# yardenas/ethz-safe-learning

Measured on NVIDIA B200. Metric: CEM-MPC plans/sec (PointGoal1 shape; ensemble transitions/sec alongside), higher is better.
Workload: dtype bf16

## Files before the change

ethz-safe-learning_b200/csrc/rollout_tc.cu:

```cuda
#include <cuda_bf16.h>

#include <cstdlib>
#include <type_traits>

#include "common.cuh"
#include "internal.h"
#include "rollout_params.cuh"
#include "tc_head.cuh"
#include "tc_ptx.cuh"

namespace simba {

#ifdef SIMBA_TC_TIMELINE
#define TL(ev)                                                                                   \
  do {                                                                                           \
    if (tl_who >= 0 && blockIdx.x == 0)                                                          \
      prm.timeline[(tl_who * 64 + tl_t) * 64 + (ev)] = clock64();  \
  } while (0)
#else
#define TL(ev) do { } while (0)
#endif

namespace {

constexpr int kU = 128;
constexpr int kMaxO = 60;
constexpr int kAtomBytes = 128 * 128;
constexpr int kBoundThreads = 640;

struct TileInfo {
  int32_t member, k0, count, valid;
};

template <int NB, int kThreads>
struct NoiseSmem {
  uint4* base;
  __device__ __forceinline__ uint4 get4(int b) const { return base[b * kThreads]; }
  __device__ __forceinline__ void put4(int b, uint4 v) { base[b * kThreads] = v; }
  __device__ __forceinline__ void put4_dyn(int b, uint4 v) { base[b * kThreads] = v; }
};
template <int NB>
struct NoiseRegs {
  uint4 v[NB];
  __device__ __forceinline__ uint4 get4(int b) const { return v[b]; }
  __device__ __forceinline__ void put4(int b, uint4 x) { v[b] = x; }
  __device__ __forceinline__ void put4_dyn(int b, uint4 x) {
#pragma unroll
    for (int i = 0; i < NB; ++i)
      if (i == b) v[i] = x;
  }
};

struct AStoreTmem {
  uint32_t t_a;
  __device__ __forceinline__ void store8(int k0, uint32_t p0, uint32_t p1, uint32_t p2, uint32_t p3) const {
    const uint32_t pk[4] = {p0, p1, p2, p3};
    tmem_st<4>(t_a + (uint32_t)(k0 >> 1), pk);
  }
};

struct AStorePair {
  uint32_t t_a;
  uint32_t peer_slot;
  uint32_t buf_off;
  uint32_t peer_bar;
  __device__ __forceinline__ void store8(int k0, uint32_t p0, uint32_t p1, uint32_t p2, uint32_t p3) const {
    const uint32_t pk[4] = {p0, p1, p2, p3};
    tmem_st<4>(t_a + (uint32_t)(k0 >> 1), pk);
    st_async_v4(peer_slot + buf_off, p0, p1, p2, p3, peer_bar);
  }
};

}

template <int NTILES, int Q, bool PAIR, bool TRAJ>
__device__ __forceinline__ void rollout_tc_body(const RolloutParams& prm) {
  static_assert(!PAIR || (NTILES == 1 && Q == 4), "the pair variant is the one-tile latency configuration");
  static_assert(!(PAIR && TRAJ), "the trajectory form has no pair variant");
  constexpr int kTileThreads = Q * 128;
  constexpr int kTileWarps = Q * 4;
  constexpr int kEpiThreads = NTILES * kTileThreads;
  constexpr int kEpiWarps = kEpiThreads / 32;
  constexpr int OW = (PAIR ? 32 : 64) / Q;
  constexpr int NSL = PAIR ? 2 * Q : Q;
  constexpr int NB = OW / 8;
  constexpr int HCOLS = 128 / Q;
  constexpr int kTmemCols = NTILES * 256;
  constexpr bool kPark = NTILES > 1;
  constexpr int kBarAcc = 2, kBarA = 2 + NTILES, kBarPart = 2 + 2 * NTILES, kBarFree = 2 + 3 * NTILES;
  extern __shared__ __align__(1024) uint8_t smem_raw[];
  const RowGeom& g = prm.g;
  const int L = prm.L;
  const int H = g.H;
  const int O = g.O, A = g.A;
  const int warp = threadIdx.x >> 5, lane = threadIdx.x & 31;
  const uint32_t crank = PAIR ? cluster_ctarank() : 0u;
  const int n_items = (prm.n_tiles + NTILES - 1) / NTILES;
  const int cta_item0 = PAIR ? (int)(blockIdx.x >> 1) : (int)blockIdx.x;
  const int n_ctas = PAIR ? (int)(gridDim.x >> 1) : (int)gridDim.x;
  const bool l0_pad_bias = (O + A + 2 <= 64);
  constexpr int n_quarters = 4;
  constexpr int tile_bar_threads = Q * 128 + 32;

  const uint32_t w_bytes = kAtomBytes + (uint32_t)L * 2 * kAtomBytes;
  uint8_t* w_smem = smem_raw;
  uint8_t* biask_smem = w_smem + w_bytes;
  uint8_t* ones_smem = biask_smem + (L + 1) * 4096;
  float* scale_smem = reinterpret_cast<float*>(ones_smem + 4096);
  float* pen_smem = scale_smem + 128;
  const int nparts = TRAJ ? 1 : 1 + prm.scorer.n_constraints;
  float* part_smem = pen_smem + kHeadParts * 64;
  const int part_buf_floats = NTILES * NSL * nparts * 128;
  uint4* xch_smem = reinterpret_cast<uint4*>(part_smem + (PAIR ? 2 : 1) * part_buf_floats);
  uint4* noise_smem = xch_smem + (PAIR ? 2 * Q * 128 : 0);
  uint32_t* rs_smem = reinterpret_cast<uint32_t*>(noise_smem + (kPark ? NB * kEpiThreads : 0));
  uint64_t* bars = reinterpret_cast<uint64_t*>(rs_smem + NTILES * 8 * 128);
  uint32_t* tmem_slot = reinterpret_cast<uint32_t*>(bars + 1 + NTILES + 2);
  TileInfo* tinfo = reinterpret_cast<TileInfo*>(tmem_slot + 2);
  uint64_t* seed_sh = reinterpret_cast<uint64_t*>(tinfo + NTILES);
  int32_t* w_state_sh = reinterpret_cast<int32_t*>(seed_sh + 1);

  const uint32_t bar_w = smem_u32(&bars[0]);

#ifdef SIMBA_TC_TIMELINE
#define TLK(k) do { if (blockIdx.x == 0 && threadIdx.x == 0) { prm.timeline[(3 * 64) * 64 + (k)] = clock64(); \
    unsigned long long gt_; asm volatile("mov.u64 %0, %%globaltimer;" : "=l"(gt_)); \
    prm.timeline[(3 * 64 + 10 + prm.iteration) * 64 + (k)] = (long long)gt_; } } while (0)
#else
#define TLK(k) do { } while (0)
#endif
  TLK(0);
  pdl_launch_dependents();
  auto item_member = [&](int item) {
    int wm = -1;
    for (int q = 0; q < NTILES; ++q)
      if (item * NTILES + q < prm.n_tiles && prm.tiles[item * NTILES + q].count > 0) wm = prm.tiles[item * NTILES + q].member;
    return wm;
  };
  auto stage_weights = [&](int wm) {
    const uint8_t* wsrc = reinterpret_cast<const uint8_t*>(prm.w_bf16) + (size_t)wm * prm.w_bf16_member_bytes;
    const uint32_t bk_bytes = (uint32_t)(L + 1) * 4096u;
    mbar_expect_tx(bar_w, w_bytes + bk_bytes);
    uint32_t off = 0;
    for (int l = 0; l <= L; ++l) {
      const uint32_t nb = (l == 0) ? kAtomBytes : 2 * kAtomBytes;
      bulk_g2s(smem_u32(w_smem + off), wsrc + off, nb, bar_w);
      off += nb;
    }
    bulk_g2s(smem_u32(biask_smem), reinterpret_cast<const uint8_t*>(prm.bias_k16) + (size_t)wm * bk_bytes,
             bk_bytes, bar_w);
    w_state_sh[0] = wm;
    w_state_sh[1] += 1;
  };
  if (threadIdx.x == 0) {
    mbar_init(bar_w, 1);
#pragma unroll
    for (int j = 0; j < NTILES; ++j) {
      mbar_init(smem_u32(&bars[1 + j]), 1);
    }
    if (PAIR) {
      mbar_init(smem_u32(&bars[1 + NTILES]), 1);
      mbar_init(smem_u32(&bars[2 + NTILES]), 1);
    }
    fence_barrier_init();
    w_state_sh[0] = -1;
    w_state_sh[1] = 0;
    const int wm = cta_item0 < n_items ? item_member(cta_item0) : -1;
    if (wm >= 0) stage_weights(wm);
  }
  auto load_tile = [&](int ti) {
    TileInfo info{0, 0, 0, 0};
    if (ti < prm.n_tiles) {
      const Tile t = prm.tiles[ti];
      info.member = t.member; info.k0 = t.k0; info.count = t.count;
      info.valid = t.count > 0 ? 1 : 0;
    }
    return info;
  };
  if (threadIdx.x < NTILES) tinfo[threadIdx.x] = load_tile(cta_item0 * NTILES + threadIdx.x);
  if (warp == 0) tmem_alloc(smem_u32(tmem_slot), kTmemCols);
  if (warp < kEpiWarps) {
    for (int i = threadIdx.x; i < 1024; i += kEpiThreads) {
      const int byte = i * 4;
      const bool first = ((byte & 255) < 128) && ((byte & 15) == 0);
      reinterpret_cast<uint32_t*>(ones_smem)[i] = first ? 0x3F803F80u : 0u;
    }
    fence_proxy_async();
    if constexpr (TRAJ) {
      head_tables_init(scale_smem, pen_smem, prm.tc_scale_a, prm.tc_scale_b, simba_scorer_t{},
                       l0_pad_bias ? O + A : -1, threadIdx.x, kEpiThreads);
    } else {
      head_tables_init(scale_smem, pen_smem, prm.tc_scale_a, prm.tc_scale_b, prm.scorer,
                       l0_pad_bias ? O + A : -1, threadIdx.x, kEpiThreads);
    }
  }
  if (PAIR && threadIdx.x == 0) {
    const uint32_t per_step = crank == 0 ? (uint32_t)(kEpiThreads * 4 * nparts) : 0u;
    mbar_expect_tx(smem_u32(&bars[2 + NTILES]), per_step + (uint32_t)(kEpiThreads * 16));
    const uint32_t b0 = per_step + (1 < H ? (uint32_t)(kEpiThreads * 16) : 0u);
    if (b0 != 0u) mbar_expect_tx(smem_u32(&bars[1 + NTILES]), b0);
  }
  tc_fence_before();
  __syncthreads();
  if (PAIR) cluster_sync_all();
  tc_fence_after();
  const uint32_t tmem_base = *tmem_slot;
  TLK(1);
  constexpr bool kLateWait = PAIR;
  if (!kLateWait) pdl_wait_prior_grid();
  TLK(2);
  if (threadIdx.x == 0) *seed_sh = prm.seed_ptr ? *prm.seed_ptr : prm.seed;
  auto tile_active = [&](const TileInfo& t) {
    if (prm.active == nullptr) return true;
    const int m = g.rows_per_state[t.member];
    bool any = false;
    for (int s = t.k0 / m; s <= (t.k0 + t.count - 1) / m; ++s) any = any || prm.active[s] != 0;
    return any;
  };
  auto late_gate = [&](const TileInfo& t) {
    if (!kLateWait) return true;
    pdl_wait_prior_grid();
    return tile_active(t);
  };
  uint32_t ph = 0;

#pragma unroll 1
  for (int item = cta_item0; item < n_items; item += n_ctas) {
  if (threadIdx.x < NTILES) {
    TileInfo info = tinfo[threadIdx.x];
    if (item != cta_item0) info = load_tile(item * NTILES + threadIdx.x);
    if (!kLateWait && info.valid) info.valid = tile_active(info) ? 1 : 0;
    tinfo[threadIdx.x] = info;
  }
  __syncthreads();
  bool any_valid = false;
  int member = -1;
#pragma unroll
  for (int j = 0; j < NTILES; ++j)
    if (tinfo[j].valid) { any_valid = true; member = tinfo[j].member; }
  if (threadIdx.x == 0 && any_valid && member != w_state_sh[0]) {
    if (w_state_sh[1] > 0) mbar_wait(bar_w, (uint32_t)(w_state_sh[1] - 1) & 1u);
    stage_weights(member);
  }
  __syncthreads();

  if (any_valid) {
    if (warp >= kEpiWarps + NTILES) {
      const int j = warp - kEpiWarps - NTILES;
      const TileInfo tis = tinfo[j];
      auto xbytes = [&](int t) -> uint32_t {
        return (crank == 0 ? (uint32_t)(kEpiThreads * 4 * nparts) : 0u) + (t + 1 < H ? (uint32_t)(kEpiThreads * 16) : 0u);
      };
      const uint32_t xbar = smem_u32(&bars[1 + NTILES]);
      if (PAIR && tis.valid && crank != 0 && late_gate(tis)) {
        for (int ts = -1; ts + 1 < H; ++ts) {
          mbar_wait(xbar + 8u * ((uint32_t)ts & 1u), (uint32_t)((ts + 1) >> 1) & 1u);
          if (lane == 0 && xbytes(ts + 2) != 0u) mbar_expect_tx(xbar + 8u * ((uint32_t)ts & 1u), xbytes(ts + 2));
        }
      }
      if (!TRAJ && tis.valid && crank == 0) {
        const simba_scorer_t& sc = prm.scorer;
        const bool done_first = objective_done_first(prm.objective);
        uint32_t* my_rs = rs_smem + j * 8 * 128 + lane;
        const float* part_tile0 = part_smem + (j * NSL * nparts) * 128;
#pragma unroll 1
        for (int i = 0; i < n_quarters; ++i) {
          const int row = lane + 32 * i;
#pragma unroll
          for (int f = 0; f < 7; ++f) my_rs[f * 128 + 32 * i] = 0u;
          my_rs[7 * 128 + 32 * i] = row < tis.count ? (uint32_t)decode_row(g, tis.member, tis.k0 + row).out : 0xffffffffu;
        }
        const bool live = late_gate(tis);
        for (int ts = -1; live && ts < H; ++ts) {
          named_bar_sync_n(kBarPart + j, tile_bar_threads);
          const float* part_tile = part_tile0;
          if (PAIR) {
            mbar_wait(xbar + 8u * ((uint32_t)ts & 1u), (uint32_t)((ts + 1) >> 1) & 1u);
            if (lane == 0 && ts + 2 < H) mbar_expect_tx(xbar + 8u * ((uint32_t)ts & 1u), xbytes(ts + 2));
            part_tile += (ts & 1) * part_buf_floats;
          }
#pragma unroll 1
          for (int i = 0; i < n_quarters; ++i) {
            uint32_t* q = my_rs + 32 * i;
            float nd, nc;
            head_combine<NSL>(sc, part_tile + lane + 32 * i, nparts, nd, nc);
            if (ts < 0) {
              q[4 * 128] = __float_as_uint(nd);
              q[5 * 128] = __float_as_uint(nc);
            } else {
              RowScore rs;
              rs.cum = __uint_as_float(q[0]);
              rs.costsum = __uint_as_float(q[128]);
              rs.cmask = (uint64_t)q[2 * 128] | ((uint64_t)q[3 * 128] << 32);
              rs.dist = __uint_as_float(q[4 * 128]);
              rs.cost = __uint_as_float(q[5 * 128]);
              rs.done = q[6 * 128] != 0u;
              head_score_step(rs, sc, done_first, ts, nd, nc);
              q[0] = __float_as_uint(rs.cum);
              q[128] = __float_as_uint(rs.costsum);
              q[2 * 128] = (uint32_t)rs.cmask;
              q[3 * 128] = (uint32_t)(rs.cmask >> 32);
              q[4 * 128] = __float_as_uint(rs.dist);
              q[5 * 128] = __float_as_uint(rs.cost);
              q[6 * 128] = rs.done ? 1u : 0u;
            }
          }
          if (ts + 1 < H) named_bar_arrive_n(kBarFree + j, tile_bar_threads);
        }
        if (live && prm.row_return != nullptr) {
#pragma unroll 1
          for (int i = 0; i < n_quarters; ++i) {
            const uint32_t* q = my_rs + 32 * i;
            const uint32_t slot = q[7 * 128];
            if (slot != 0xffffffffu) {
              prm.row_return[slot] = __uint_as_float(q[0]);
              prm.row_costmask[slot] = (uint64_t)q[2 * 128] | ((uint64_t)q[3 * 128] << 32);
              prm.row_costsum[slot] = __uint_as_float(q[128]);
            }
          }
        }
      }
    } else if (warp >= kEpiWarps) {
      const int j = warp - kEpiWarps;
      if (tinfo[j].valid) {
        const uint32_t bar_acc = smem_u32(&bars[1 + j]);
        const uint32_t d_tmem = tmem_base + (uint32_t)j * 128;
        const uint32_t a_tmem = tmem_base + (uint32_t)(NTILES * 192 + j * 64);
        const uint64_t ones_desc = umma_desc_k16_noswizzle(smem_u32(ones_smem));
        mbar_wait(bar_w, (uint32_t)(w_state_sh[1] - 1) & 1u);
#ifdef SIMBA_TC_TIMELINE
        const int tl_who = (j == 0 && lane == 0) ? 2 : -1;
#endif
        const bool live = late_gate(tinfo[j]);
        for (int t = 0; live && t < H; ++t) {
#ifdef SIMBA_TC_TIMELINE
          const int tl_t = t;
#endif
          for (int layer = 0; layer <= L; ++layer) {
            named_bar_sync_n(kBarA + j, tile_bar_threads);
            tc_fence_after();
            TL(2 * layer);
            if (elect_one()) {
              const uint32_t woff = (layer == 0) ? 0u : (uint32_t)(kAtomBytes + (layer - 1) * 2 * kAtomBytes);
              const uint64_t b0 = umma_desc_sw128(smem_u32(w_smem + woff));
#pragma unroll
              for (int k = 0; k < 4; ++k)
                umma_bf16_ts(d_tmem, a_tmem + (uint32_t)k * 8, b0 + (uint64_t)((k * 32) >> 4), kIdesc, k > 0 ? 1u : 0u);
              if (layer > 0) {
#pragma unroll
                for (int k = 4; k < 8; ++k)
                  umma_bf16_ts(d_tmem, a_tmem + (uint32_t)k * 8, b0 + (uint64_t)((kAtomBytes + (k - 4) * 32) >> 4),
                               kIdesc, 1u);
              }
              if (layer > 0 || !l0_pad_bias)
                umma_bf16(d_tmem, ones_desc, umma_desc_k16_noswizzle(smem_u32(biask_smem + layer * 4096)), kIdesc, 1u);
              umma_commit(bar_acc);
            }
            TL(2 * layer + 1);
            __syncwarp();
            mbar_wait(bar_acc, ph);
            ph ^= 1;
            tc_fence_before();
            named_bar_arrive_n(kBarAcc + j, tile_bar_threads);
          }
        }
      }
    } else {
      const int j = warp / kTileWarps;
      const int wl = warp - j * kTileWarps;
      const int cgp = wl >> 2;
      const int r = (wl & 3) * 32 + lane;
      const TileInfo ti = tinfo[j];
      if (ti.valid) {
        const bool row_ok = r < ti.count;
        const RowId id = decode_row(g, ti.member, ti.k0 + (row_ok ? r : 0));
        const uint32_t lane_base = tmem_base + ((uint32_t)((wl & 3) * 32) << 16);
        const uint32_t t_acc = lane_base + (uint32_t)j * 128;
        const uint32_t t_a = lane_base + (uint32_t)(NTILES * 192 + j * 64);
        const float* act_ptr = prm.actions + ((int64_t)id.s * g.N + id.i_global) * prm.action_stride;
        const simba_scorer_t& sc = prm.scorer;

        HeadCtx hc;
        hc.t_acc = t_acc;
        hc.t_state = lane_base + (uint32_t)(NTILES * 128 + j * 64);
        hc.o_base = (PAIR ? (int)crank * 32 : 0) + cgp * OW;
        hc.O = O; hc.A = A;
        hc.slice_bits = TRAJ ? 0u : head_slice_bits<OW>(sc, hc.o_base);
        hc.n_constraints = TRAJ ? 0 : sc.n_constraints;
        hc.scale_smem = scale_smem;
        hc.pen_smem = pen_smem;
        float* part_slot0 = part_smem + ((j * NSL + (int)crank * Q + cgp) * nparts) * 128 + r;
        hc.part = part_slot0 + (PAIR ? part_buf_floats : 0);
        typename std::conditional<PAIR, AStorePair, AStoreTmem>::type astore;
        astore.t_a = t_a;
        const uint32_t my_xbar = smem_u32(&bars[1 + NTILES]);
        const uint32_t peer_xbar = PAIR ? cluster_map_u32(my_xbar, crank ^ 1u) : 0u;
        const bool keeps_score = !TRAJ && (!PAIR || crank == 0);
        const uint32_t part_remote0 = (PAIR && crank != 0) ? cluster_map_u32(smem_u32(part_slot0), 0u) : 0u;
        if constexpr (PAIR) {
          astore.peer_slot = cluster_map_u32(smem_u32(xch_smem + cgp * 128 + r), crank ^ 1u);
          astore.buf_off = (uint32_t)(Q * 128 * sizeof(uint4));
          astore.peer_bar = peer_xbar + 8u;
          if (crank != 0) {
            hc.part_remote = part_remote0 + (uint32_t)(part_buf_floats * sizeof(float));
            hc.part_mbar = peer_xbar + 8u;
          }
        }
        auto exchange = [&](int t, bool next_step) {
          if constexpr (PAIR) {
            const uint32_t b = (uint32_t)t & 1u;
            if (next_step) {
              mbar_wait(my_xbar + 8u * b, (uint32_t)((t + 1) >> 1) & 1u);
              const uint4 v = xch_smem[(b * Q + cgp) * 128 + r];
              const uint32_t pk[4] = {v.x, v.y, v.z, v.w};
              tmem_st<4>(t_a + (uint32_t)((((int)crank ^ 1) * 32 + cgp * 8) >> 1), pk);
            }
          }
        };
        const float* s0_ptr = prm.states + (prm.state_per_row ? id.r_global : (int64_t)id.s) * prm.state_stride;
        typename std::conditional<TRAJ, TrajSink, NoTraj>::type sink{};
        if constexpr (TRAJ) {
          sink.row = row_ok ? prm.traj_out + id.out * (int64_t)(H + 1) * O : nullptr;
          sink.O = O;
        }

#ifdef SIMBA_TC_TIMELINE
        const int tl_who = (j == 0 && lane == 0) ? (wl == 0 ? 0 : (wl == kTileWarps - 1 ? 1 : -1)) : -1;
        int tl_t = 0;
#endif
        auto publish_a = [&]() {
          tmem_st_wait();
          tc_fence_before();
          named_bar_arrive_n(kBarA + j, tile_bar_threads);
        };
        auto wait_accumulator = [&]() {
          named_bar_sync_n(kBarAcc + j, tile_bar_threads);
          tc_fence_after();
        };

        const bool owns_actions = TRAJ ? (O < hc.o_base + OW) && (O + A > hc.o_base)
                                       : (O >= hc.o_base) && (O < hc.o_base + OW);
        float act_pf[4] = {0.f, 0.f, 0.f, 0.f};
        auto prefetch_actions = [&](int tn) {
          if (owns_actions && row_ok && tn < H) {
#pragma unroll
            for (int a = 0; a < 4; ++a)
              if (a < A) act_pf[a] = act_ptr[tn * A + a];
          }
        };

        typename std::conditional<kPark, NoiseSmem<NB, kEpiThreads>, NoiseRegs<NB>>::type noise;
        if constexpr (kPark) noise.base = noise_smem + threadIdx.x;
#pragma unroll
        for (int b = 0; b < NB; ++b) noise.put4(b, make_uint4(0u, 0u, 0u, 0u));
        const uint32_t c3_noise = (uint32_t)id.s | (kStreamNoise << 28);
        const uint32_t row32 = (uint32_t)id.r_global;
        const float* eps_row = prm.eps == nullptr ? nullptr
            : prm.eps + ((int64_t)id.s * H * ((int64_t)g.P * g.N) + id.r_global) * O;
        const int64_t eps_step = (int64_t)g.P * g.N * O;
        const uint64_t seed64 = *seed_sh;
        const uint2 key = make_uint2((uint32_t)seed64, (uint32_t)(seed64 >> 32));
        const uint32_t c2_base = (uint32_t)prm.iteration << 16;
        auto make_noise = [&](int b, int t) {
          const int o0 = hc.o_base + b * 8;
          if (o0 >= O) return;
          uint4 z;
          if (eps_row != nullptr) {
            z = external_noise8_bf16(eps_row + t * eps_step, o0, O);
          } else {
#ifdef SIMBA_TC_TIMELINE
            {
              PhiloxState p{(uint32_t)(o0 >> 3), row32, (uint32_t)t | c2_base, c3_noise, key.x, key.y};
              TL(50);
              philox_rounds<10>(p);
              if (p.c0 == 0x12345u) TL(53);
              TL(51);
              z = philox_finish_noise8_bf16(p);
              if (z.x == 0x12345u) TL(53);
              TL(52);
            }
#else
            z = philox_noise8_bf16(key, (uint32_t)(o0 >> 3), row32, (uint32_t)t | c2_base, c3_noise);
#endif
            if (o0 + 8 > O) z = mask_noise8(z, o0, O);
          }
          noise.put4_dyn(b, z);
        };
        float s0v[8];
        if constexpr (PAIR) {
#pragma unroll
          for (int i = 0; i < 8; ++i) s0v[i] = (row_ok && hc.o_base + i < O) ? s0_ptr[hc.o_base + i] : 0.0f;
        }
        const bool live = late_gate(ti);
        if (live) {
        prefetch_actions(0);
        if constexpr (PAIR) head_first_pass_vals(hc, astore, s0v, act_pf);
        else head_first_pass<OW>(hc, astore, s0_ptr, row_ok, act_pf, sink);
        prefetch_actions(1);
        exchange(-1, true);
        publish_a();
        TLK(3);
        if (keeps_score) named_bar_arrive_n(kBarPart + j, tile_bar_threads);

        PhiloxState ps{0u, 0u, 0u, 0u, 0u, 0u};
        for (int t = 0; t < H; ++t) {
#ifdef SIMBA_TC_TIMELINE
          tl_t = t;
#endif
          TL(0);
          if (owns_actions) {
            if constexpr (TRAJ) head_store_own_actions<OW>(hc, act_pf);
            else head_store_actions(hc, act_pf);
          }
          prefetch_actions(t + 2);
          for (int l = 0; l < L; ++l) {
            wait_accumulator();
            TL(1 + l * 4);
            {
              constexpr int NLD = HCOLS / 32;
              uint32_t v[NLD][32];
#pragma unroll
              for (int i = 0; i < NLD; ++i) tmem_ld<32>(t_acc + (uint32_t)(cgp * HCOLS + i * 32), v[i]);
              tmem_ld_wait();
#pragma unroll
              for (int i = 0; i < NLD; ++i) {
                uint32_t pk[16];
#pragma unroll
                for (int q = 0; q < 16; ++q)
                  pk[q] = pack_relu_bf16(__uint_as_float(v[i][2 * q]), __uint_as_float(v[i][2 * q + 1]));
                tmem_st<16>(t_a + (uint32_t)((cgp * HCOLS + i * 32) / 2), pk);
              }
            }
            TL(2 + l * 4);
            publish_a();
            TL(3 + l * 4);
            if (prm.sampling_propagation) {
              if (NTILES == 1 && L >= 2 * NB && eps_row == nullptr) {
                const int b = l >> 1, o0 = hc.o_base + b * 8;
                if (b < NB && o0 < O) {
                  if ((l & 1) == 0) {
                    ps = PhiloxState{(uint32_t)(o0 >> 3), row32, (uint32_t)t | c2_base, c3_noise, key.x, key.y};
                    philox_rounds<10>(ps);
                  } else {
                    uint4 z = philox_finish_noise8_bf16(ps);
                    if (o0 + 8 > O) z = mask_noise8(z, o0, O);
                    noise.put4_dyn(b, z);
                  }
                }
              } else {
                if (l < NB) make_noise(l, t);
                if (l == L - 1)
                  for (int b = L; b < NB; ++b) make_noise(b, t);
              }
            }
            TL(4 + l * 4);
          }

          wait_accumulator();
          if (keeps_score) named_bar_sync_n(kBarFree + j, tile_bar_threads);
          TL(40);
          if constexpr (PAIR) {
            hc.part = part_slot0 + (t & 1) * part_buf_floats;
            astore.buf_off = (uint32_t)((t & 1) * Q * 128 * sizeof(uint4));
            astore.peer_bar = peer_xbar + 8u * ((uint32_t)t & 1u);
            if (crank != 0) {
              hc.part_remote = part_remote0 + (uint32_t)((t & 1) * part_buf_floats * sizeof(float));
              hc.part_mbar = astore.peer_bar;
            }
          }
          if constexpr (TRAJ) {
            if (sink.row != nullptr) sink.row += O;
          }
          if (prm.sampling_propagation) head_step_pass<OW, true>(hc, noise, astore, t + 1 < H, sink);
          else head_step_pass<OW, false>(hc, noise, astore, t + 1 < H, sink);
          TL(41);
          exchange(t, t + 1 < H);
          if (t + 1 < H) publish_a();
          if (keeps_score) named_bar_arrive_n(kBarPart + j, tile_bar_threads);
          TL(42);
        }
        TLK(6);
        }
      }
    }
  }

  tc_fence_before();
  __syncthreads();
  tc_fence_after();
  }

  if (threadIdx.x == 0 && w_state_sh[1] > 0) mbar_wait(bar_w, (uint32_t)(w_state_sh[1] - 1) & 1u);
  tc_fence_before();
  __syncthreads();
  TLK(4);
  if (warp == 0) tmem_dealloc(tmem_base, kTmemCols);
  TLK(5);
}

template <int NTILES, int Q, bool PAIR>
__global__ void __launch_bounds__(kBoundThreads, 1) rollout_tc_kernel(const RolloutParams prm) {
  rollout_tc_body<NTILES, Q, PAIR, false>(prm);
}

template <int NTILES, int Q>
__global__ void __launch_bounds__(kBoundThreads, 1) unfold_tc_kernel(const RolloutParams prm) {
  rollout_tc_body<NTILES, Q, false, true>(prm);
}

static size_t tc_smem_bytes(int L, int ntiles, int q, int nparts, bool pair = false) {
  size_t b = (size_t)kAtomBytes + (size_t)L * 2 * kAtomBytes;
  b += (size_t)(L + 1) * 4096 + 4096;
  b += 128 * sizeof(float);
  b += kHeadParts * 64 * sizeof(float);
  b += (size_t)ntiles * q * nparts * 128 * sizeof(float) * (pair ? 4 : 1);
  if (pair) b += (size_t)2 * q * 128 * sizeof(uint4);
  if (ntiles > 1)
    b += (size_t)(64 / q / 8) * (ntiles * q * 128) * sizeof(uint4);
  b += (size_t)8 * ntiles * 128 * sizeof(uint32_t);
  b += (3 + ntiles) * sizeof(uint64_t) + 2 * sizeof(uint32_t) + ntiles * sizeof(TileInfo) + sizeof(uint64_t) + 2 * sizeof(int32_t);
  return b + 1024;
}

constexpr size_t kMaxSmem = 227 * 1024;

bool rollout_tc_supported(int O, int A, int L, int U) {
  return U >= 1 && U <= kU && O >= 1 && O <= kMaxO && O + A <= 64 && A <= 4 && L >= 1 &&
         tc_smem_bytes(L, 1, 4, kHeadParts) + 1024 <= kMaxSmem;
}

bool rollout_tc_two_tiles_fit(int L, int n_constraints) {
  return tc_smem_bytes(L, 2, 2, 1 + n_constraints) + 1024 <= kMaxSmem;
}

bool rollout_tc_pair_fits(int L, int n_constraints) {
  return tc_smem_bytes(L, 1, 4, 1 + n_constraints, true) + 1024 <= kMaxSmem;
}

template <int NTILES, int Q, bool PAIR, bool TRAJ>
static cudaError_t launch_variant(const RolloutParams& prm, cudaStream_t stream) {
  void (*kern)(const RolloutParams) = rollout_tc_kernel<NTILES, Q, PAIR>;
  if constexpr (TRAJ) kern = unfold_tc_kernel<NTILES, Q>;
  const size_t smem = tc_smem_bytes(prm.L, NTILES, Q, TRAJ ? 1 : 1 + prm.scorer.n_constraints, PAIR);
  const int n_items = (prm.n_tiles + NTILES - 1) / NTILES;
  const int sms = prm.n_sms;
  if (sms <= 0) return cudaErrorInvalidValue;
  const int grid = PAIR ? 2 * n_items : (n_items < sms ? n_items : sms);
  return launch_kernel(kern, grid, NTILES * Q * 128 + 64 * NTILES, smem, stream, PAIR ? 2 : 1, prm.pdl, prm);
}

cudaError_t launch_rollout_tc(const RolloutParams& prm, cudaStream_t stream) {
  if (prm.traj_out == nullptr) {
    switch (prm.kernel) {
      case RolloutKernel::kTcOneCta: return launch_variant<1, 4, false, false>(prm, stream);
      case RolloutKernel::kTcPair: return launch_variant<1, 4, true, false>(prm, stream);
      case RolloutKernel::kTcTwoTile: return launch_variant<2, 2, false, false>(prm, stream);
      default: return cudaErrorInvalidValue;
    }
  }
  switch (prm.kernel) {
    case RolloutKernel::kTcOneCta: return launch_variant<1, 4, false, true>(prm, stream);
    case RolloutKernel::kTcTwoTile: return launch_variant<2, 2, false, true>(prm, stream);
    default: return cudaErrorInvalidValue;
  }
}

}
```

Baseline: 2661.

## Double-buffer TMEM accumulators and split one-tile MMA into column halves

For the one-tile variants, the accumulator and activation regions in tensor memory are double-buffered by GEMM parity, and each layer's MMA is split into two 64-column halves with separate commit barriers. A new relay warp turns the mbarrier completions into per-half named-barrier arrivals, so each half of the epilogue warps can start draining its columns while the other half's MMA is still running. The intent is to overlap MMA issue with the epilogue's TMEM load, ReLU and store between layers. In exchange it takes all 512 TMEM columns, adds an extra warp and more barrier traffic, and makes the phase and parity bookkeeping considerably more complex.

```diff
diff --git a/ethz-safe-learning_b200/csrc/rollout_tc.cu b/ethz-safe-learning_b200/csrc/rollout_tc.cu
--- a/ethz-safe-learning_b200/csrc/rollout_tc.cu
+++ b/ethz-safe-learning_b200/csrc/rollout_tc.cu
@@ -85,9 +85,14 @@
   constexpr int NSL = PAIR ? 2 * Q : Q;
   constexpr int NB = OW / 8;
   constexpr int HCOLS = 128 / Q;
-  constexpr int kTmemCols = NTILES * 256;
+  constexpr bool kDbl = NTILES == 1;
+  static_assert(!kDbl || Q == 4, "the one-tile variants split the columns into halves of two column groups");
+  constexpr int kTmemCols = 512;
+  constexpr uint32_t kStateCol = kDbl ? 256 : NTILES * 128;
+  constexpr uint32_t kACol = kDbl ? 320 : NTILES * 192;
   constexpr bool kPark = NTILES > 1;
   constexpr int kBarAcc = 2, kBarA = 2 + NTILES, kBarPart = 2 + 2 * NTILES, kBarFree = 2 + 3 * NTILES;
+  constexpr int kBarAccHi = 6, kBarAHi = 7;
   extern __shared__ __align__(1024) uint8_t smem_raw[];
   const RowGeom& g = prm.g;
   const int L = prm.L;
@@ -101,6 +106,7 @@
   const bool l0_pad_bias = (O + A + 2 <= 64);
   constexpr int n_quarters = 4;
   constexpr int tile_bar_threads = Q * 128 + 32;
+  constexpr int half_bar_threads = Q * 64 + 32;
 
   const uint32_t w_bytes = kAtomBytes + (uint32_t)L * 2 * kAtomBytes;
   uint8_t* w_smem = smem_raw;
@@ -115,7 +121,7 @@
   uint4* noise_smem = xch_smem + (PAIR ? 2 * Q * 128 : 0);
   uint32_t* rs_smem = reinterpret_cast<uint32_t*>(noise_smem + (kPark ? NB * kEpiThreads : 0));
   uint64_t* bars = reinterpret_cast<uint64_t*>(rs_smem + NTILES * 8 * 128);
-  uint32_t* tmem_slot = reinterpret_cast<uint32_t*>(bars + 1 + NTILES + 2);
+  uint32_t* tmem_slot = reinterpret_cast<uint32_t*>(bars + 1 + NTILES + 2 + (kDbl ? 1 : 0));
   TileInfo* tinfo = reinterpret_cast<TileInfo*>(tmem_slot + 2);
   uint64_t* seed_sh = reinterpret_cast<uint64_t*>(tinfo + NTILES);
   int32_t* w_state_sh = reinterpret_cast<int32_t*>(seed_sh + 1);
@@ -158,6 +164,7 @@
     for (int j = 0; j < NTILES; ++j) {
       mbar_init(smem_u32(&bars[1 + j]), 1);
     }
+    if (kDbl) mbar_init(smem_u32(&bars[3 + NTILES]), 1);
     if (PAIR) {
       mbar_init(smem_u32(&bars[1 + NTILES]), 1);
       mbar_init(smem_u32(&bars[2 + NTILES]), 1);
@@ -245,7 +252,22 @@
   __syncthreads();
 
   if (any_valid) {
-    if (warp >= kEpiWarps + NTILES) {
+    if (kDbl && warp == kEpiWarps + 2 * NTILES) {
+      if (tinfo[0].valid && late_gate(tinfo[0])) {
+        const uint32_t bar_lo = smem_u32(&bars[1]), bar_hi = smem_u32(&bars[3 + NTILES]);
+        for (int t = 0; t < H; ++t) {
+          for (int layer = 0; layer <= L; ++layer) {
+            mbar_wait(layer < L ? bar_lo : bar_hi, ph);
+            tc_fence_before();
+            named_bar_arrive_n(kBarAcc, half_bar_threads);
+            mbar_wait(bar_hi, ph);
+            ph ^= 1;
+            tc_fence_before();
+            named_bar_arrive_n(kBarAccHi, half_bar_threads);
+          }
+        }
+      }
+    } else if (warp >= kEpiWarps + NTILES) {
       const int j = warp - kEpiWarps - NTILES;
       const TileInfo tis = tinfo[j];
       auto xbytes = [&](int t) -> uint32_t {
@@ -325,13 +347,84 @@
       if (tinfo[j].valid) {
         const uint32_t bar_acc = smem_u32(&bars[1 + j]);
         const uint32_t d_tmem = tmem_base + (uint32_t)j * 128;
-        const uint32_t a_tmem = tmem_base + (uint32_t)(NTILES * 192 + j * 64);
+        const uint32_t a_tmem = tmem_base + (uint32_t)(kACol + j * 64);
         const uint64_t ones_desc = umma_desc_k16_noswizzle(smem_u32(ones_smem));
         mbar_wait(bar_w, (uint32_t)(w_state_sh[1] - 1) & 1u);
 #ifdef SIMBA_TC_TIMELINE
         const int tl_who = (j == 0 && lane == 0) ? 2 : -1;
 #endif
         const bool live = late_gate(tinfo[j]);
+        if constexpr (kDbl) {
+          const uint32_t bar_acc_hi = smem_u32(&bars[3 + NTILES]);
+          constexpr uint32_t kIdesc64 = umma_idesc_n(64u), kIdesc32 = umma_idesc_n(32u);
+          uint32_t par = 0;
+          auto mma4 = [&](uint32_t d, uint32_t a, uint64_t b, uint32_t idesc, int kb) {
+#pragma unroll
+            for (int k = 0; k < 4; ++k)
+              umma_bf16_ts(d, a + (uint32_t)(kb + k) * 8, b + (uint64_t)(((kb ? kAtomBytes : 0) + k * 32) >> 4), idesc,
+                           (kb + k) > 0 ? 1u : 0u);
+          };
+          auto mma_bias = [&](uint32_t d, uint32_t bias_sm, uint32_t col, uint32_t idesc) {
+            umma_bf16(d, ones_desc, umma_desc_k16_noswizzle(bias_sm + col * 32), idesc, 1u);
+          };
+          for (int t = 0; live && t < H; ++t) {
+#ifdef SIMBA_TC_TIMELINE
+            const int tl_t = t;
+#endif
+            {
+              const uint32_t d = d_tmem + par * 128, a = a_tmem + par * 64;
+              const uint64_t b = umma_desc_sw128(smem_u32(w_smem));
+              const uint32_t bias_sm = smem_u32(biask_smem);
+              named_bar_sync_n(kBarA, half_bar_threads);
+              named_bar_sync_n(kBarAHi, half_bar_threads);
+              tc_fence_after();
+              TL(0);
+              if (elect_one()) {
+                mma4(d, a, b, kIdesc64, 0);
+                if (!l0_pad_bias) mma_bias(d, bias_sm, 0u, kIdesc64);
+                umma_commit(bar_acc);
+                mma4(d + 64, a, b + (uint64_t)((64 * 128) >> 4), kIdesc64, 0);
+                if (!l0_pad_bias) mma_bias(d + 64, bias_sm, 64u, kIdesc64);
+                umma_commit(bar_acc_hi);
+              }
+              TL(1);
+              __syncwarp();
+              par ^= 1;
+            }
+            for (int layer = 1; layer <= L; ++layer) {
+              const uint32_t d = d_tmem + par * 128, a = a_tmem + par * 64;
+              const bool own_head = PAIR && layer == L;
+              const uint32_t c0 = own_head ? crank * 32 : 0u, c1 = own_head ? 64u + crank * 32 : 64u;
+              const uint32_t idesc = own_head ? kIdesc32 : kIdesc64;
+              const uint64_t bw = umma_desc_sw128(smem_u32(w_smem + kAtomBytes + (layer - 1) * 2 * kAtomBytes));
+              const uint64_t b0 = bw + (uint64_t)((c0 * 128) >> 4), b1 = bw + (uint64_t)((c1 * 128) >> 4);
+              const uint32_t bias_sm = smem_u32(biask_smem + layer * 4096);
+              named_bar_sync_n(kBarA, half_bar_threads);
+              tc_fence_after();
+              TL(2 * layer);
+              if (elect_one()) {
+                mma4(d + c0, a, b0, idesc, 0);
+                mma4(d + c1, a, b1, idesc, 0);
+              }
+              TL(2 * layer + 1);
+              __syncwarp();
+              named_bar_sync_n(kBarAHi, half_bar_threads);
+              tc_fence_after();
+              TL(20 + 2 * layer);
+              if (elect_one()) {
+                mma4(d + c0, a, b0, idesc, 4);
+                mma_bias(d + c0, bias_sm, c0, idesc);
+                umma_commit(bar_acc);
+                mma4(d + c1, a, b1, idesc, 4);
+                mma_bias(d + c1, bias_sm, c1, idesc);
+                umma_commit(bar_acc_hi);
+              }
+              TL(21 + 2 * layer);
+              __syncwarp();
+              par ^= 1;
+            }
+          }
+        } else
         for (int t = 0; live && t < H; ++t) {
 #ifdef SIMBA_TC_TIMELINE
           const int tl_t = t;
@@ -376,13 +469,13 @@
         const RowId id = decode_row(g, ti.member, ti.k0 + (row_ok ? r : 0));
         const uint32_t lane_base = tmem_base + ((uint32_t)((wl & 3) * 32) << 16);
         const uint32_t t_acc = lane_base + (uint32_t)j * 128;
-        const uint32_t t_a = lane_base + (uint32_t)(NTILES * 192 + j * 64);
+        const uint32_t t_a = lane_base + (uint32_t)(kACol + j * 64);
         const float* act_ptr = prm.actions + ((int64_t)id.s * g.N + id.i_global) * prm.action_stride;
         const simba_scorer_t& sc = prm.scorer;
 
         HeadCtx hc;
         hc.t_acc = t_acc;
-        hc.t_state = lane_base + (uint32_t)(NTILES * 128 + j * 64);
+        hc.t_state = lane_base + (uint32_t)(kStateCol + j * 64);
         hc.o_base = (PAIR ? (int)crank * 32 : 0) + cgp * OW;
         hc.O = O; hc.A = A;
         hc.slice_bits = TRAJ ? 0u : head_slice_bits<OW>(sc, hc.o_base);
@@ -413,7 +506,7 @@
               mbar_wait(my_xbar + 8u * b, (uint32_t)((t + 1) >> 1) & 1u);
               const uint4 v = xch_smem[(b * Q + cgp) * 128 + r];
               const uint32_t pk[4] = {v.x, v.y, v.z, v.w};
-              tmem_st<4>(t_a + (uint32_t)((((int)crank ^ 1) * 32 + cgp * 8) >> 1), pk);
+              tmem_st<4>(astore.t_a + (uint32_t)((((int)crank ^ 1) * 32 + cgp * 8) >> 1), pk);
             }
           }
         };
@@ -428,15 +521,20 @@
         const int tl_who = (j == 0 && lane == 0) ? (wl == 0 ? 0 : (wl == kTileWarps - 1 ? 1 : -1)) : -1;
         int tl_t = 0;
 #endif
+        static_assert(!kDbl || kBarAccHi - kBarAcc == kBarAHi - kBarA, "one offset selects both barriers of a half");
+        const int bar_off = kDbl ? (cgp >= Q / 2 ? kBarAHi - kBarA : 0) : j;
+        const int bar_acc_mine = kBarAcc + bar_off, bar_a_mine = kBarA + bar_off;
+        const int hand_off_threads = kDbl ? half_bar_threads : tile_bar_threads;
         auto publish_a = [&]() {
           tmem_st_wait();
           tc_fence_before();
-          named_bar_arrive_n(kBarA + j, tile_bar_threads);
+          named_bar_arrive_n(bar_a_mine, hand_off_threads);
         };
         auto wait_accumulator = [&]() {
-          named_bar_sync_n(kBarAcc + j, tile_bar_threads);
+          named_bar_sync_n(bar_acc_mine, hand_off_threads);
           tc_fence_after();
         };
+        auto gemm_par = [&](int t, int l) { return (uint32_t)(t * (L + 1) + l) & 1u; };
 
         const bool owns_actions = TRAJ ? (O < hc.o_base + OW) && (O + A > hc.o_base)
                                        : (O >= hc.o_base) && (O < hc.o_base + OW);
@@ -520,7 +618,7 @@
               constexpr int NLD = HCOLS / 32;
               uint32_t v[NLD][32];
 #pragma unroll
-              for (int i = 0; i < NLD; ++i) tmem_ld<32>(t_acc + (uint32_t)(cgp * HCOLS + i * 32), v[i]);
+              for (int i = 0; i < NLD; ++i) tmem_ld<32>(t_acc + (kDbl ? gemm_par(t, l) * 128 : 0u) + (uint32_t)(cgp * HCOLS + i * 32), v[i]);
               tmem_ld_wait();
 #pragma unroll
               for (int i = 0; i < NLD; ++i) {
@@ -528,7 +626,7 @@
 #pragma unroll
                 for (int q = 0; q < 16; ++q)
                   pk[q] = pack_relu_bf16(__uint_as_float(v[i][2 * q]), __uint_as_float(v[i][2 * q + 1]));
-                tmem_st<16>(t_a + (uint32_t)((cgp * HCOLS + i * 32) / 2), pk);
+                tmem_st<16>(t_a + (kDbl ? (gemm_par(t, l) ^ 1u) * 64 : 0u) + (uint32_t)((cgp * HCOLS + i * 32) / 2), pk);
               }
             }
             TL(2 + l * 4);
@@ -571,6 +669,10 @@
           if constexpr (TRAJ) {
             if (sink.row != nullptr) sink.row += O;
           }
+          if constexpr (kDbl) {
+            hc.t_acc = t_acc + gemm_par(t, L) * 128;
+            astore.t_a = t_a + (gemm_par(t, L) ^ 1u) * 64;
+          }
           if (prm.sampling_propagation) head_step_pass<OW, true>(hc, noise, astore, t + 1 < H, sink);
           else head_step_pass<OW, false>(hc, noise, astore, t + 1 < H, sink);
           TL(41);
@@ -618,7 +720,7 @@
   if (ntiles > 1)
     b += (size_t)(64 / q / 8) * (ntiles * q * 128) * sizeof(uint4);
   b += (size_t)8 * ntiles * 128 * sizeof(uint32_t);
-  b += (3 + ntiles) * sizeof(uint64_t) + 2 * sizeof(uint32_t) + ntiles * sizeof(TileInfo) + sizeof(uint64_t) + 2 * sizeof(int32_t);
+  b += (3 + ntiles + (ntiles == 1 ? 1 : 0)) * sizeof(uint64_t) + 2 * sizeof(uint32_t) + ntiles * sizeof(TileInfo) + sizeof(uint64_t) + 2 * sizeof(int32_t);
   return b + 1024;
 }
 
@@ -646,7 +748,7 @@
   const int sms = prm.n_sms;
   if (sms <= 0) return cudaErrorInvalidValue;
   const int grid = PAIR ? 2 * n_items : (n_items < sms ? n_items : sms);
-  return launch_kernel(kern, grid, NTILES * Q * 128 + 64 * NTILES, smem, stream, PAIR ? 2 : 1, prm.pdl, prm);
+  return launch_kernel(kern, grid, NTILES * Q * 128 + 64 * NTILES + (NTILES == 1 ? 32 : 0), smem, stream, PAIR ? 2 : 1, prm.pdl, prm);
 }
 
 cudaError_t launch_rollout_tc(const RolloutParams& prm, cudaStream_t stream) {
```

Measured after the change: 2865, median of 6. 7.7% higher.
